# RQLuo/CDLNet-video

Measured on AMD Instinct MI355X. Metric: Mpix/s denoised (fwd+bwd) at K=30,M=64,P=7, higher is better.
Workload: dtype f32 (split-bf16 x3 MFMA, fp32 accumulate, fp32 storage)

## Files before the change

### cdlnet-video_amd/csrc/cdl_fused2d.hip

```cpp
#include <atomic>
#include <cstdlib>
#include <type_traits>
#include <mutex>
#include <utility>
#include <vector>

#include "cdl_common.h"


namespace {

typedef __attribute__((ext_vector_type(8))) __bf16 bf16x8;
typedef __attribute__((ext_vector_type(4))) __bf16 bf16x4;
typedef __attribute__((ext_vector_type(16))) float f32x16;

constexpr int WX = 2;
constexpr int RB = 8;
constexpr int TW = 32 * WX;
constexpr int HALO = 3;
constexpr int RTW = TW + 2 * HALO;
constexpr int RTC = RTW + 2;
constexpr int LDS_W = 32 * 64 * 16;
constexpr int LDS_TAU = 64 * 4;

// ... 115 lines not shown
#endif
#ifndef CDL_FAT_ST_AUX
#define CDL_FAT_ST_AUX 0
#endif
__device__ __forceinline__ __amdgpu_buffer_rsrc_t fat_rsrc(const float *base, size_t img_floats)
{
    return __builtin_amdgcn_make_buffer_rsrc(const_cast<float *>(base), 0, (int)(img_floats * 4), 0x00020000);
}
__device__ __forceinline__ float buf_ld(__amdgpu_buffer_rsrc_t r, int voff, int soff)
{
    return __builtin_bit_cast(float, __builtin_amdgcn_raw_buffer_load_b32(r, voff, soff, CDL_FAT_LD_AUX));
}
__device__ __forceinline__ void buf_st(float v, __amdgpu_buffer_rsrc_t r, int voff, int soff)
{
    __builtin_amdgcn_raw_buffer_store_b32(__builtin_bit_cast(unsigned, v), r, voff, soff, CDL_FAT_ST_AUX);
}
constexpr int OOB = 0x7fff0000;

enum { LAY_NCHW = 0, LAY_BLK = 1, LAY_BLK16 = 2 };
typedef __attribute__((ext_vector_type(4))) unsigned u32x4;
typedef __attribute__((ext_vector_type(2))) unsigned u32x2;

__host__ __device__ inline size_t blk_image_elems(int M, int H, int W) { return (size_t)H * ((W + 31) / 32) * M * 32; }
template <int LAY> __host__ __device__ inline size_t lay_image_bytes(int M, int H, int W)
{
    return LAY == LAY_NCHW ? (size_t)M * H * W * 4 : blk_image_elems(M, H, W) * (LAY == LAY_BLK ? 4 : 2);
}

__device__ __forceinline__ __amdgpu_buffer_rsrc_t uniform_rsrc(const void *base, size_t bytes)
{
    const unsigned long long a = reinterpret_cast<unsigned long long>(base);
    const unsigned lo = __builtin_amdgcn_readfirstlane((unsigned)a);
    const unsigned hi = __builtin_amdgcn_readfirstlane((unsigned)(a >> 32));
    void *b = reinterpret_cast<void *>(((unsigned long long)hi << 32) | lo);
    return __builtin_amdgcn_make_buffer_rsrc(b, 0, __builtin_amdgcn_readfirstlane((int)bytes), 0x00020000);
}

__device__ __forceinline__ float bf16_round(float v) { return (float)(__bf16)v; }

template <int MT>
__device__ __forceinline__ void blk16_load_raw(u32x2 (&z)[MT][4], __amdgpu_buffer_rsrc_t rs, int voff)
{
#pragma unroll
    for (int R = 0; R < MT; ++R)
#pragma unroll
        for (int q = 0; q < 4; ++q)
            z[R][q] = __builtin_bit_cast(u32x2, __builtin_amdgcn_raw_buffer_load_b64(rs, voff, (8 * R + 2 * q) * 32 * 8, CDL_FAT_LD_AUX));
}
__device__ __forceinline__ float blk16_decode(const u32x2 &u, int e)
{
    const unsigned w = (e & 2) ? u.y : u.x;
    return __builtin_bit_cast(float, (e & 1) ? (w & 0xffff0000u) : (w << 16));
}

template <int LAY, int MT>
__device__ __forceinline__ void blk_load(float (&z)[MT][16], __amdgpu_buffer_rsrc_t rs, int voff)
{
    constexpr int EB = LAY == LAY_BLK ? 16 : 8;
#pragma unroll
    for (int R = 0; R < MT; ++R)
#pragma unroll
        for (int q = 0; q < 4; ++q) {
            const int soff = (8 * R + 2 * q) * 32 * EB;
            if constexpr (LAY == LAY_BLK) {
                typedef __attribute__((ext_vector_type(4))) float f32x4;
                const f32x4 f = __builtin_bit_cast(f32x4, __builtin_amdgcn_raw_buffer_load_b128(rs, voff, soff, CDL_FAT_LD_AUX));
                z[R][4 * q + 0] = f.x; z[R][4 * q + 1] = f.y; z[R][4 * q + 2] = f.z; z[R][4 * q + 3] = f.w;
            } else {
                const u32x2 u = __builtin_bit_cast(u32x2, __builtin_amdgcn_raw_buffer_load_b64(rs, voff, soff, CDL_FAT_LD_AUX));
                z[R][4 * q + 0] = __builtin_bit_cast(float, u.x << 16);
                z[R][4 * q + 1] = __builtin_bit_cast(float, u.x & 0xffff0000u);
                z[R][4 * q + 2] = __builtin_bit_cast(float, u.y << 16);
                z[R][4 * q + 3] = __builtin_bit_cast(float, u.y & 0xffff0000u);
            }
        }
}
template <int LAY>
__device__ __forceinline__ void blk_store4(float a0, float a1, float a2, float a3, __amdgpu_buffer_rsrc_t rs, int voff, int quad_pair)
{
    constexpr int EB = LAY == LAY_BLK ? 16 : 8;
    const int soff = quad_pair * 32 * EB;
    if constexpr (LAY == LAY_BLK) {
        typedef __attribute__((ext_vector_type(4))) float f32x4;
        const f32x4 f = {a0, a1, a2, a3};
        __builtin_amdgcn_raw_buffer_store_b128(__builtin_bit_cast(u32x4, f), rs, voff, soff, CDL_FAT_ST_AUX);
    } else {
        u32x2 u;
        u.x = (__builtin_bit_cast(unsigned, a0) >> 16) | (__builtin_bit_cast(unsigned, a1) & 0xffff0000u);
        u.y = (__builtin_bit_cast(unsigned, a2) >> 16) | (__builtin_bit_cast(unsigned, a3) & 0xffff0000u);
        __builtin_amdgcn_raw_buffer_store_b64(u, rs, voff, soff, CDL_FAT_ST_AUX);
    }
}

template <int N>
struct LaneTransposeSum {
    static __device__ __forceinline__ float run(const float (&v)[N], int c)
    {
        constexpr int n = N / 2;
        const bool up = (c & n) != 0;
        float w[n];
#pragma unroll
        for (int k = 0; k < n; ++k) {
            const float keep = up ? v[k + n] : v[k];
            const float send = up ? v[k] : v[k + n];
            w[k] = keep + __shfl_xor(send, n, 64);
        }
        return LaneTransposeSum<n>::run(w, c);
    }
};
template <>
struct LaneTransposeSum<1> {
    static __device__ __forceinline__ float run(const float (&v)[1], int) { return v[0]; }
};
template <int N>
__device__ __forceinline__ float lane_transpose_sum(const float (&v)[N], int c)
{
    float r = LaneTransposeSum<N>::run(v, c);
    if (N == 16) r += __shfl_xor(r, 16, 64);
    return r;
}

__device__ __forceinline__ float wave_shr1(float v)
{
    return __builtin_bit_cast(float, __builtin_amdgcn_update_dpp(0, __builtin_bit_cast(int, v), 0x138, 0xf, 0xf, true));
}
__device__ __forceinline__ float upper_half_to_lower(float v)
{
    float lo = 0.0f;
    asm volatile("s_nop 1\n\tv_permlane32_swap_b32 %0, %1\n\ts_nop 1" : "+v"(v), "+v"(lo));
    return lo;
}
__device__ __forceinline__ float col2im_row(const float (&rv)[4], int h)
{
    const float r4 = upper_half_to_lower(rv[0]);
    const float r5 = upper_half_to_lower(rv[1]);
    const float r6 = upper_half_to_lower(rv[2]);
    const bool lo = h == 0;
    float s = lo ? r6 : 0.0f;
    s = wave_shr1(s) + (lo ? r5 : 0.0f);
    s = wave_shr1(s) + (lo ? r4 : 0.0f);
    s = wave_shr1(s) + (lo ? rv[3] : 0.0f);
    s = wave_shr1(s) + (lo ? rv[2] : 0.0f);
    s = wave_shr1(s) + (lo ? rv[1] : 0.0f);
    s = wave_shr1(s) + (lo ? rv[0] : 0.0f);
    return s;
}

template <int MT, int PREC, int MODE, int LIN, int LOUT, bool DA = false, int WY = 2>
__global__ __launch_bounds__(Shape<WY>::NT) void k_stage(FusedParams p)
{
    using G = Shape<WY>;
    constexpr int NW = G::NW, NT = G::NT, TH = G::TH, RTH = G::RTH, PITCH = G::PITCH, COPY = G::COPY, SLAB = G::SLAB;
    constexpr int LDS_RT = G::LDS_RT, LDS_RSUM = G::LDS_RSUM, LDS_STAGE = G::LDS_STAGE, LDS_DA_THIN = G::LDS_DA_THIN;
    static_assert(!DA || (MODE == MODE_BWD && TH == GW_TH), "dA_k rides in the reverse stage, on k_wgrad2d's 64 x 16 tiles");
    extern __shared__ __attribute__((aligned(16))) unsigned char smem[];
    __bf16 *rt = reinterpret_cast<__bf16 *>(smem);
    float *rsum_all = reinterpret_cast<float *>(smem + LDS_RT);
    const uint4 *wl = reinterpret_cast<const uint4 *>(smem + LDS_RT + LDS_RSUM);
    float *tau_s = reinterpret_cast<float *>(smem + LDS_RT + LDS_RSUM + LDS_W);
    float *tacc_s = tau_s + 64;
    __bf16 *thin2 = reinterpret_cast<__bf16 *>(smem + LDS_STAGE);
    __bf16 *imgs2 = reinterpret_cast<__bf16 *>(smem + LDS_STAGE + LDS_DA_THIN);

    constexpr int M = 32 * MT;
    constexpr int FA = MT * 4, FB = 4 * MT;
    constexpr int NFRAG = (PREC != 1 ? 2 : 1) * (FA + FB);
    constexpr int NSTG = G::NSTG;
    const int tid = threadIdx.x, lane = tid & 63, wid = tid >> 6;
    const int wxi = wid % WX, wyi = wid / WX;
    const int c = lane & 31, h = lane >> 5;
    const size_t HW = (size_t)p.H * p.W;
    const int numTiles = p.N * p.tilesY * p.tilesX;

    {
        uint4 *z4 = reinterpret_cast<uint4 *>(smem);
        for (int i = tid; i < (LDS_RT + LDS_RSUM) / 16; i += NT) z4[i] = make_uint4(0, 0, 0, 0);
        uint4 *wdst = reinterpret_cast<uint4 *>(smem + LDS_RT + LDS_RSUM);
        if (PREC != 1) {
            for (int i = tid; i < NFRAG * 64; i += NT) wdst[i] = p.frags[i];
        } else {
            for (int i = tid; i < FA * 64; i += NT) wdst[i] = p.frags[i];
            for (int i = tid; i < FB * 64; i += NT) wdst[FA * 64 + i] = p.frags[2 * FA * 64 + i];
        }
    }
    float stg[NSTG];
    auto stage_load = [&](int t) {
        int bid = p.rev ? numTiles - 1 - t : t;
        const int txi = bid % p.tilesX; bid /= p.tilesX;
        const int tyi = bid % p.tilesY;
        const int n = bid / p.tilesY;
        const float *rimg = p.r + (size_t)n * HW;
#pragma unroll
        for (int k = 0; k < NSTG; ++k) {
            const int i = tid + k * NT;
            const int yy = i / RTW, xx = i % RTW;
            const int gy = tyi * TH - HALO + yy, gx = txi * TW - HALO + xx;
            float v = 0.0f;
            if (i < RTH * RTW && t < numTiles && !CDL_DBG(p.dbg, 8) && gy >= 0 && gy < p.H && gx >= 0 && gx < p.W)
                v = rimg[(size_t)gy * p.W + gx];
            stg[k] = v;
        }
    };
    auto stage_store = [&]() {
#pragma unroll
        for (int k = 0; k < NSTG; ++k) {
            const int i = tid + k * NT;
            if (i >= RTH * RTW) continue;
            const int yy = i / RTW, xx = i % RTW;
            const __bf16 hh = (__bf16)stg[k];
            const __bf16 ll = (__bf16)(stg[k] - (float)hh);
#pragma unroll
            for (int q = 0; q < 4; ++q)
                if (yy - q >= 0) {
                    rt[(0 * 4 + q) * COPY + xx * PITCH + (yy - q)] = hh;
                    if (PREC != 1) rt[(1 * 4 + q) * COPY + xx * PITCH + (yy - q)] = ll;
                }
        }
    };
    constexpr int NSTG2 = DA ? (GW_RTH * RTW + NT - 1) / NT : 1;
    float stg2[NSTG2];
    auto stage2_load = [&](int t) {
        int bid = p.rev ? numTiles - 1 - t : t;
        const int txi = bid % p.tilesX; bid /= p.tilesX;
        const int tyi = bid % p.tilesY;
        const int n = bid / p.tilesY;
        const float *timg = p.r2 + (t < numTiles ? (size_t)n * HW : 0);
#pragma unroll
        for (int k = 0; k < NSTG2; ++k) {
            const int i = tid + k * NT;
            const int yy = i / RTW, xx = i % RTW;
            const int gy = tyi * TH - HALO + yy, gx = txi * TW - HALO + xx;
            const bool ok = i < GW_RTH * RTW && t < numTiles && gy >= 0 && gy < p.H && gx >= 0 && gx < p.W;
            const float v = timg[ok ? (size_t)gy * p.W + gx : 0];
            stg2[k] = ok ? v : 0.0f;
        }
    };
    auto stage2_store = [&]() {
#pragma unroll
        for (int k = 0; k < NSTG2; ++k) {
            const int i = tid + k * NT;
            if (i >= GW_RTH * RTW) continue;
            const int yy = i / RTW, xx = i % RTW;
            const __bf16 hh = (__bf16)stg2[k];
            const __bf16 ll = (__bf16)(stg2[k] - (float)hh);
#pragma unroll
            for (int sft = 0; sft < 4; ++sft)
                if (xx - sft >= 0) {
                    thin2[(0 * 4 + sft) * TCOPY + yy * TPITCH + xx - sft] = hh;
                    if (PREC != 1) thin2[(1 * 4 + sft) * TCOPY + yy * TPITCH + xx - sft] = ll;
                }
        }
    };
    f32x16 dacc[DA ? MT : 1][2];
    if constexpr (DA) {
#pragma unroll
        for (int R = 0; R < MT; ++R)
#pragma unroll
            for (int tt = 0; tt < 2; ++tt)
#pragma unroll
                for (int v = 0; v < 16; ++v) dacc[R][tt][v] = 0.0f;
        for (int i = tid; i < LDS_DA_THIN / 16; i += NT) reinterpret_cast<uint4 *>(thin2)[i] = make_uint4(0, 0, 0, 0);
        stage2_load(blockIdx.x);
    }
    stage_load(blockIdx.x);
    __syncthreads();
    stage_store();
    if constexpr (DA) stage2_store();

    constexpr int OFF_AH = 0;
    constexpr int OFF_AL = FA;
    constexpr int OFF_BH = (PREC != 1 ? 2 * FA : FA);
    constexpr int OFF_BL = 2 * FA + FB;
    constexpr bool WREG = G::WREG;
    bf16x8 wreg[WREG ? NFRAG : 1];
    if constexpr (WREG) {
#pragma unroll
        for (int f = 0; f < NFRAG; ++f) wreg[f] = __builtin_bit_cast(bf16x8, wl[f * 64 + lane]);
    }
    auto wfrag = [&](int f) __attribute__((always_inline)) {
        if constexpr (WREG) return wreg[f];
        else return __builtin_bit_cast(bf16x8, wl[f * 64 + lane]);
    };

    const int xl = wxi * 32 + c;
    float *rsum = rsum_all + ((wxi & 1) + 2 * (wyi & 1)) * SLAB;
    const bool has_base = (MODE == MODE_FWD) || (MODE == MODE_BWD && p.zin != nullptr);
    const int hw4 = (int)HW * 4;

#pragma unroll 1
    for (int t = blockIdx.x; t < numTiles; t += gridDim.x) {
    const int tile = p.rev ? numTiles - 1 - t : t;
    int bid = tile;
    const int txi = bid % p.tilesX; bid /= p.tilesX;
    const int tyi = bid % p.tilesY;
    const int n = bid / p.tilesY;
    const int tx0 = txi * TW, ty0 = tyi * TH;
    const int x = tx0 + xl;
    if (MODE != MODE_BWD && tid < M) tau_s[tid] = p.tau[(size_t)n * M + tid];
    __syncthreads();
    if (MODE != MODE_BWD) stage_load(t + gridDim.x);

    float ring[7][4];
#pragma unroll
    for (int i = 0; i < 7; ++i)
#pragma unroll
        for (int j = 0; j < 4; ++j) ring[i][j] = 0.0f;
    float tsum[MT * 16];
#pragma unroll
    for (int i = 0; i < MT * 16; ++i) tsum[i] = 0.0f;
    const bool tau_neg = MODE != MODE_BWD && __ballot(lane < M && !(tau_s[lane] >= 0.0f)) != 0ull;
    float taur[MT * 16];
    if (MODE != MODE_BWD) {
#pragma unroll
        for (int R = 0; R < MT; ++R)
#pragma unroll
            for (int qv = 0; qv < 4; ++qv) {
                const float4 t4 = *reinterpret_cast<const float4 *>(&tau_s[32 * R + 8 * qv + 4 * h]);
                taur[16 * R + 4 * qv + 0] = t4.x; taur[16 * R + 4 * qv + 1] = t4.y;
                taur[16 * R + 4 * qv + 2] = t4.z; taur[16 * R + 4 * qv + 3] = t4.w;
            }
    }

    const bool xok = x < p.W;
    const size_t img_in = lay_image_bytes<LIN>(M, p.H, p.W), img_out = lay_image_bytes<LOUT>(M, p.H, p.W);
    const __amdgpu_buffer_rsrc_t rs_in = uniform_rsrc(
        has_base ? (const char *)p.zin + (size_t)n * img_in : (const char *)p.zout, has_base ? img_in : 0);
    unsigned *const map_n = p.map ? p.map + ((size_t)n * 4 + 2 * h) * HW : nullptr;
    const __amdgpu_buffer_rsrc_t rs_out = uniform_rsrc((const char *)p.zout + (size_t)n * img_out, img_out);
    const int lane_off = (int)((4 * h) * HW + x) * 4;
    const int XB = (p.W + 31) / 32, xb = (tx0 >> 5) + wxi;
    constexpr int EB_IN = LIN == LAY_BLK16 ? 8 : 16, EB_OUT = LOUT == LAY_BLK16 ? 8 : 16;
    const int lane_blk_in = (h * 32 + c) * EB_IN, lane_blk_out = (h * 32 + c) * EB_OUT;

#pragma unroll 1
    for (int b = 0; b < RB; ++b) {
        const int yl = wyi * RB + b;
        const int y = ty0 + yl;
        const bool valid = xok && (y < p.H);
        const int voff = valid ? lane_off + y * p.W * 4 : OOB;
        const int blk = (y * XB + xb) * (M / 4) * 32;
        const int voff_in = LIN == LAY_NCHW ? voff : (valid ? blk * EB_IN + lane_blk_in : OOB);
        const int voff_st = CDL_DBG(p.dbg, 1) ? OOB : (LOUT == LAY_NCHW ? voff : (valid ? blk * EB_OUT + lane_blk_out : OOB));

        float zc[MT][16];
        u32x2 zr[MT][4];
        if (MODE != MODE_FIRST && LIN == LAY_BLK16) {
            blk16_load_raw<MT>(zr, rs_in, voff_in);
        } else if (MODE != MODE_FIRST && CDL_DBG(p.dbg, 16)) {
#pragma unroll
            for (int R = 0; R < MT; ++R)
#pragma unroll
                for (int v = 0; v < 16; ++v) zc[R][v] = 0.25f;
        } else if (MODE != MODE_FIRST && LIN != LAY_NCHW) {
            blk_load<LIN, MT>(zc, rs_in, voff_in);
        } else if (MODE != MODE_FIRST) {
#pragma unroll
            for (int R = 0; R < MT; ++R)
#pragma unroll
                for (int v = 0; v < 16; ++v) {
                    const int soff = (32 * R + 8 * (v >> 2) + (v & 3)) * hw4;
                    zc[R][v] = buf_ld(rs_in, voff, soff);
                }
        }
        unsigned sup = 0, sgb = 0;
        if (MODE == MODE_BWD && valid) {
            sup = map_n[(size_t)y * p.W + x];
            sgb = map_n[HW + (size_t)y * p.W + x];
        }

        const int q = b & 3, e = yl - q;
        bf16x8 rh[4], rl[4];
#pragma unroll
        for (int ks = 0; ks < 4; ++ks) {
            const int col = xl + 2 * ks + h;
            const __bf16 *ph = rt + (0 * 4 + q) * COPY + col * PITCH + e;
            const bf16x4 a0 = *reinterpret_cast<const bf16x4 *>(ph);
            const bf16x4 a1 = *reinterpret_cast<const bf16x4 *>(ph + 4);
            rh[ks] = __builtin_shufflevector(a0, a1, 0, 1, 2, 3, 4, 5, 6, 7);
            if (PREC != 1) {
                const __bf16 *pl = rt + (1 * 4 + q) * COPY + col * PITCH + e;
                const bf16x4 b0 = *reinterpret_cast<const bf16x4 *>(pl);
                const bf16x4 b1 = *reinterpret_cast<const bf16x4 *>(pl + 4);
                rl[ks] = __builtin_shufflevector(b0, b1, 0, 1, 2, 3, 4, 5, 6, 7);
            }
        }

        __builtin_amdgcn_sched_barrier(0);
        f32x16 acc[MT];
#pragma unroll
        for (int R = 0; R < MT; ++R)
#pragma unroll
            for (int v = 0; v < 16; ++v) acc[R][v] = 0.0f;
        if CDL_DBG(p.dbg, 4) {
#pragma unroll
            for (int R = 0; R < MT; ++R) acc[R][0] = (float)rh[0][0] + (float)rl[1][1];
        } else {
            bf16x8 wh[2][MT], wlo[2][MT];
#pragma unroll
            for (int R = 0; R < MT; ++R) {
                wh[0][R] = wfrag(OFF_AH + R * 4);
                if (PREC != 1) wlo[0][R] = wfrag(OFF_AL + R * 4);
            }
#pragma unroll
            for (int ks = 0; ks < 4; ++ks) {
                const int cu = ks & 1, nx = cu ^ 1;
                if (ks + 1 < 4) {
#pragma unroll
                    for (int R = 0; R < MT; ++R) {
                        wh[nx][R] = wfrag(OFF_AH + R * 4 + ks + 1);
                        if (PREC != 1) wlo[nx][R] = wfrag(OFF_AL + R * 4 + ks + 1);
                    }
                }
                if (PREC != 1) {
#pragma unroll
                    for (int R = 0; R < MT; ++R) acc[R] = __builtin_amdgcn_mfma_f32_32x32x16_bf16(wlo[cu][R], rh[ks], acc[R], 0, 0, 0);
#pragma unroll
                    for (int R = 0; R < MT; ++R) acc[R] = __builtin_amdgcn_mfma_f32_32x32x16_bf16(wh[cu][R], rl[ks], acc[R], 0, 0, 0);
                    if (PREC == 2) {
#pragma unroll
                        for (int R = 0; R < MT; ++R) acc[R] = __builtin_amdgcn_mfma_f32_32x32x16_bf16(wlo[cu][R], rl[ks], acc[R], 0, 0, 0);
                    }
                }
#pragma unroll
                for (int R = 0; R < MT; ++R) acc[R] = __builtin_amdgcn_mfma_f32_32x32x16_bf16(wh[cu][R], rh[ks], acc[R], 0, 0, 0);
            }
        }

        __builtin_amdgcn_sched_barrier(0);
        auto epilogue = [&](auto general_shrink) {
#pragma unroll
        for (int R = 0; R < MT; ++R)
#pragma unroll
            for (int v = 0; v < 16; ++v) {
                const int chl = 32 * R + 8 * (v >> 2) + (v & 3);
                float zz;
                float zbase = 0.0f;
                if (MODE != MODE_FIRST) zbase = LIN == LAY_BLK16 ? blk16_decode(zr[R][v >> 2], v & 3) : zc[R][v];
                if (MODE == MODE_BWD) {
                    const bool on = (sup >> (16 * R + v)) & 1u;
                    zz = on ? zbase + acc[R][v] : 0.0f;
                    tsum[16 * R + v] += ((sgb >> (16 * R + v)) & 1u) ? zz : -zz;
                } else {
                    const float base = (MODE == MODE_FWD) ? zbase : 0.0f;
                    const float u = fmaf(p.sgn, acc[R][v], base);
                    const float tt = taur[16 * R + v];
                    const float st = decltype(general_shrink)::value ? cdl_shrink(u, tt)
                                                                     : u - __builtin_amdgcn_fmed3f(u, -tt, tt);
                    zz = CDL_DBG(p.dbg, 64) ? u : (valid ? st : 0.0f);
                }
                if (LOUT == LAY_BLK16) zz = bf16_round(zz);
                if (LOUT == LAY_NCHW) buf_st(zz, rs_out, voff_st, chl * hw4);
                acc[R][v] = zz;
            }
        };
        if (tau_neg) epilogue(std::true_type{});
        else epilogue(std::false_type{});
        if (LOUT != LAY_NCHW) {
#pragma unroll
            for (int R = 0; R < MT; ++R)
#pragma unroll
                for (int q = 0; q < 4; ++q)
                    blk_store4<LOUT>(acc[R][4 * q], acc[R][4 * q + 1], acc[R][4 * q + 2], acc[R][4 * q + 3], rs_out,
                                     voff_st, 8 * R + 2 * q);
        }
        if (MODE != MODE_BWD && map_n) {
            unsigned ws = 0, wg = 0;
#pragma unroll
            for (int R = 0; R < MT; ++R)
#pragma unroll
                for (int v = 0; v < 16; ++v) {
                    const float zz = acc[R][v];
                    ws |= (zz != 0.0f ? 1u : 0u) << (16 * R + v);
                    wg |= (__builtin_bit_cast(unsigned, zz) >> 31) << (16 * R + v);
                }
            if (valid && !CDL_DBG(p.dbg, 1)) {
                map_n[(size_t)y * p.W + x] = ws;
                map_n[HW + (size_t)y * p.W + x] = wg;
            }
        }
        if constexpr (DA) {
            __bf16 *wimg = imgs2 + (size_t)wid * (MT * 2) * IMG_ELEMS;
#pragma unroll
            for (int R = 0; R < MT; ++R)
#pragma unroll
                for (int qv = 0; qv < 4; ++qv) {
                    bf16x4 hi4, lo4;
#pragma unroll
                    for (int e = 0; e < 4; ++e) {
                        const float val = acc[R][4 * qv + e];
                        const __bf16 hh = (__bf16)val;
                        hi4[e] = hh;
                        lo4[e] = (__bf16)(val - (float)hh);
                    }
                    const int slot = (2 * qv + h) ^ ((c >> 1) & 7);
                    __bf16 *dst = wimg + (size_t)(R * 2) * IMG_ELEMS + c * 32 + slot * 4;
                    *reinterpret_cast<bf16x4 *>(dst) = hi4;
                    if (PREC != 1 && LOUT != LAY_BLK16) *reinterpret_cast<bf16x4 *>(dst + IMG_ELEMS) = lo4;
                }
            __builtin_amdgcn_fence(__ATOMIC_RELEASE, "wavefront");
            __builtin_amdgcn_wave_barrier();
#pragma unroll
            for (int kk = 0; kk < 2; ++kk) {
                bf16x8 Bh[2], Bl[2];
#pragma unroll
                for (int tt = 0; tt < 2; ++tt) {
                    const int tap = 32 * tt + c, ti = tap >> 3, tj = tap & 7;
                    const int e0 = wxi * 32 + 16 * kk + 8 * h + (tj & 4);
                    const __bf16 *ph = thin2 + (0 * 4 + (tj & 3)) * TCOPY + (yl + ti) * TPITCH + e0;
                    const bf16x4 a0 = *reinterpret_cast<const bf16x4 *>(ph);
                    const bf16x4 a1 = *reinterpret_cast<const bf16x4 *>(ph + 4);
                    Bh[tt] = __builtin_shufflevector(a0, a1, 0, 1, 2, 3, 4, 5, 6, 7);
                    if (PREC != 1) {
                        const __bf16 *pl = ph + 4 * TCOPY;
                        const bf16x4 b0 = *reinterpret_cast<const bf16x4 *>(pl);
                        const bf16x4 b1 = *reinterpret_cast<const bf16x4 *>(pl + 4);
                        Bl[tt] = __builtin_shufflevector(b0, b1, 0, 1, 2, 3, 4, 5, 6, 7);
                    }
                }
#pragma unroll
                for (int R = 0; R < MT; ++R) {
                    const int gg = (lane >> 4) & 1, qq = (lane >> 2) & 3, pp = lane & 3;
                    bf16x4 part[2][2];
#pragma unroll
                    for (int half = 0; half < 2; ++half) {
                        const int row = 16 * kk + 8 * h + 4 * half + qq;
                        const int slot = (4 * gg + pp) ^ ((row >> 1) & 7);
                        const __bf16 *src = wimg + (size_t)(R * 2) * IMG_ELEMS + row * 32 + slot * 4;
                        part[0][half] = __builtin_amdgcn_ds_read_tr16_b64_v4bf16(
                            (__attribute__((address_space(3))) bf16x4 *)(src));
                        if (PREC != 1 && LOUT != LAY_BLK16)
                            part[1][half] = __builtin_amdgcn_ds_read_tr16_b64_v4bf16(
                                (__attribute__((address_space(3))) bf16x4 *)(src + IMG_ELEMS));
                    }
                    const bf16x8 Ah = __builtin_shufflevector(part[0][0], part[0][1], 0, 1, 2, 3, 4, 5, 6, 7);
                    bf16x8 Al;
                    if (PREC != 1 && LOUT != LAY_BLK16) Al = __builtin_shufflevector(part[1][0], part[1][1], 0, 1, 2, 3, 4, 5, 6, 7);
#pragma unroll
                    for (int tt = 0; tt < 2; ++tt) {
                        if (PREC != 1) {
                            if (LOUT != LAY_BLK16) dacc[R][tt] = __builtin_amdgcn_mfma_f32_32x32x16_bf16(Al, Bh[tt], dacc[R][tt], 0, 0, 0);
                            dacc[R][tt] = __builtin_amdgcn_mfma_f32_32x32x16_bf16(Ah, Bl[tt], dacc[R][tt], 0, 0, 0);
                            if (PREC == 2 && LOUT != LAY_BLK16) dacc[R][tt] = __builtin_amdgcn_mfma_f32_32x32x16_bf16(Al, Bl[tt], dacc[R][tt], 0, 0, 0);
                        }
                        dacc[R][tt] = __builtin_amdgcn_mfma_f32_32x32x16_bf16(Ah, Bh[tt], dacc[R][tt], 0, 0, 0);
                    }
                }
            }
            __builtin_amdgcn_fence(__ATOMIC_RELEASE, "wavefront");
            __builtin_amdgcn_wave_barrier();
        }
        if (MODE == MODE_BWD && !p.do_synth) continue;
        if CDL_DBG(p.dbg, 2) { ring[0][0] += acc[0][0] + acc[MT - 1][15]; continue; }

        __builtin_amdgcn_sched_barrier(0);
        f32x16 D[2];
#pragma unroll
        for (int Rp = 0; Rp < 2; ++Rp)
#pragma unroll
            for (int v = 0; v < 16; ++v) D[Rp][v] = 0.0f;
        {
            bf16x8 bwh[2][2], bwl[2][2];
#pragma unroll
            for (int Rp = 0; Rp < 2; ++Rp) {
                bwh[0][Rp] = wfrag(OFF_BH + Rp * 2 * MT);
                if (PREC != 1) bwl[0][Rp] = wfrag(OFF_BL + Rp * 2 * MT);
            }
#pragma unroll
            for (int q = 0; q < 2 * MT; ++q) {
                const int R = q >> 1, s = q & 1, cu = q & 1, nx = cu ^ 1;
                if (q + 1 < 2 * MT) {
#pragma unroll
                    for (int Rp = 0; Rp < 2; ++Rp) {
                        bwh[nx][Rp] = wfrag(OFF_BH + Rp * 2 * MT + q + 1);
                        if (PREC != 1) bwl[nx][Rp] = wfrag(OFF_BL + Rp * 2 * MT + q + 1);
                    }
                }
                bf16x8 zh, zl;
#pragma unroll
                for (int jj = 0; jj < 8; ++jj) {
                    const float val = acc[R][8 * s + jj];
                    const __bf16 hh = (__bf16)val;
                    zh[jj] = hh;
                    if (PREC != 1 && LOUT != LAY_BLK16) zl[jj] = (__bf16)(val - (float)hh);
                }
                if (PREC != 1) {
#pragma unroll
                    for (int Rp = 0; Rp < 2; ++Rp) D[Rp] = __builtin_amdgcn_mfma_f32_32x32x16_bf16(bwl[cu][Rp], zh, D[Rp], 0, 0, 0);
                    if (LOUT != LAY_BLK16) {
#pragma unroll
                        for (int Rp = 0; Rp < 2; ++Rp) D[Rp] = __builtin_amdgcn_mfma_f32_32x32x16_bf16(bwh[cu][Rp], zl, D[Rp], 0, 0, 0);
                        if (PREC == 2) {
#pragma unroll
                            for (int Rp = 0; Rp < 2; ++Rp) D[Rp] = __builtin_amdgcn_mfma_f32_32x32x16_bf16(bwl[cu][Rp], zl, D[Rp], 0, 0, 0);
                        }
                    }
                }
#pragma unroll
                for (int Rp = 0; Rp < 2; ++Rp) D[Rp] = __builtin_amdgcn_mfma_f32_32x32x16_bf16(bwh[cu][Rp], zh, D[Rp], 0, 0, 0);
            }
        }

        __builtin_amdgcn_sched_barrier(0);
#pragma unroll
        for (int Rp = 0; Rp < 2; ++Rp)
#pragma unroll
            for (int v = 0; v < 16; ++v) {
                const int i = 4 * Rp + (v >> 2);
                if (i <= 6) ring[i][v & 3] += D[Rp][v];
            }
        {
            const float cs = col2im_row(ring[0], h);
            if (lane < 38 && !CDL_DBG(p.dbg, 32)) rsum[yl * RTW + 32 * wxi + lane] = cs;
        }
#pragma unroll
        for (int i = 0; i < 6; ++i)
#pragma unroll
            for (int jl = 0; jl < 4; ++jl) ring[i][jl] = ring[i + 1][jl];
#pragma unroll
        for (int jl = 0; jl < 4; ++jl) ring[6][jl] = 0.0f;
    }

    if (MODE != MODE_BWD || p.do_synth) {
#pragma unroll
        for (int i = 0; i < 6; ++i) {
            const float cs = col2im_row(ring[i], h);
            if (lane < 38 && !CDL_DBG(p.dbg, 32)) rsum[(wyi * RB + RB + i) * RTW + 32 * wxi + lane] = cs;
        }
    }
    if (MODE == MODE_BWD) {
        const float tacc = lane_transpose_sum(tsum, c);
        if (c < MT * 16) {
            const int R = c >> 4, v = c & 15;
            tacc_s[wid * 64 + 32 * R + 8 * (v >> 2) + 4 * h + (v & 3)] = tacc;
        }
    }
    __syncthreads();
    if (MODE == MODE_BWD) stage_load(t + gridDim.x);
    if constexpr (DA) stage2_load(t + gridDim.x);
    if (MODE == MODE_BWD && tid < M) {
        float sacc = 0.0f;
#pragma unroll
        for (int w = 0; w < NW; ++w) sacc += tacc_s[w * 64 + tid];
        p.dtau[(size_t)tile * M + tid] = sacc;
    }
    if (MODE != MODE_BWD || p.do_synth) {
        float *patch = p.patches + (size_t)tile * SLAB;
        for (int i = tid; i < SLAB; i += NT) {
            patch[i] = (rsum_all[i] + rsum_all[SLAB + i]) + (rsum_all[2 * SLAB + i] + rsum_all[3 * SLAB + i]);
            rsum_all[i] = 0.0f; rsum_all[SLAB + i] = 0.0f; rsum_all[2 * SLAB + i] = 0.0f; rsum_all[3 * SLAB + i] = 0.0f;
        }
    }
    stage_store();
    if constexpr (DA) stage2_store();
    }
    if constexpr (DA) {
        float *red = reinterpret_cast<float *>(smem);
        for (int w = 0; w < NW; ++w) {
            __syncthreads();
            if (wid == w) {
#pragma unroll
                for (int R = 0; R < MT; ++R)
#pragma unroll
                    for (int tt = 0; tt < 2; ++tt)
#pragma unroll
                        for (int v = 0; v < 16; ++v) {
                            const int ch = 32 * R + (v & 3) + 8 * (v >> 2) + 4 * h;
                            float *dstw = &red[ch * 64 + 32 * tt + c];
                            *dstw = (w == 0 ? 0.0f : *dstw) + dacc[R][tt][v];
                        }
            }
        }
        __syncthreads();
        float *dst = p.da_partial + (size_t)blockIdx.x * 2 * M * 64;
        for (int i = tid; i < M * 64; i += NT) dst[i] = red[i];
    }
}

template <int WY>
__device__ __forceinline__ float patch_sum(const float *__restrict__ patches, int n, int Y, int X,
                                           int tilesX, int tilesY)
{
    constexpr int TH = Shape<WY>::TH, SLAB = Shape<WY>::SLAB;
    const int tyc = Y / TH, txc = X / TW;
    const int ly = Y - tyc * TH, lx = X - txc * TW;
    const int hx = (lx < HALO && txc > 0) ? -1 : ((lx >= TW - HALO && txc + 1 < tilesX) ? 1 : 0);
    const int vy = (ly < HALO && tyc > 0) ? -1 : ((ly >= TH - HALO && tyc + 1 < tilesY) ? 1 : 0);
    const float *own = patches + (((size_t)n * tilesY + tyc) * tilesX + txc) * SLAB + (ly + HALO) * RTW + lx + HALO;
    const ptrdiff_t dx = (ptrdiff_t)hx * (SLAB - TW), dy = (ptrdiff_t)vy * ((ptrdiff_t)tilesX * SLAB - TH * RTW);
    float sum = 0.0f;
    if (vy < 0) {
        if (hx < 0) sum += own[dy + dx];
        sum += own[dy];
        if (hx > 0) sum += own[dy + dx];
    }
    if (hx < 0) sum += own[dx];
    sum += own[0];
    if (hx > 0) sum += own[dx];
    if (vy > 0) {
        if (hx < 0) sum += own[dy + dx];
        sum += own[dy];
        if (hx > 0) sum += own[dy + dx];
    }
    return sum;
}

template <int ASM_ROWS, int WY>
__global__ __launch_bounds__(256) void k_assemble(const float *__restrict__ patches,
                                                  const float *__restrict__ mask,
                                                  const float *__restrict__ sub, float alpha,
                                                  float *__restrict__ out, int N, int H, int W,
                                                  int tilesX, int tilesY, float *__restrict__ acc, int acc_add)
{
    const int X = blockIdx.x * 256 + threadIdx.x, n = blockIdx.z;
    if (X >= W) return;
#pragma unroll
    for (int j = 0; j < ASM_ROWS; ++j) {
        const int Y = blockIdx.y * ASM_ROWS + j;
        if (Y >= H) break;
        const size_t i = ((size_t)n * H + Y) * W + X;
        const float raw = patch_sum<WY>(patches, n, Y, X, tilesX, tilesY);
        if (acc) acc[i] = acc_add ? acc[i] + raw : raw;
        if (!out) continue;
        float sum = alpha * raw;
        if (mask) sum *= mask[i];
        if (sub) sum -= sub[i];
        out[i] = sum;
    }
}

template <int WY>
__global__ __launch_bounds__(256) void k_assemble_v4(const float *__restrict__ patches,
                                                     const float *__restrict__ mask, const float *__restrict__ sub,
                                                     float alpha, float *__restrict__ out, int N, int H, int W,
                                                     int tilesX, int tilesY, float *__restrict__ accum, int acc_add)
{
    constexpr int TH = Shape<WY>::TH, SLAB = Shape<WY>::SLAB;
    const int X = (blockIdx.x * 64 + (threadIdx.x & 63)) * 4, n = blockIdx.z;
    if (X >= W) return;
    const int txc = X / TW, lx = X - txc * TW;
// ... 1019 lines not shown
```

### cdlnet-video_amd/ops.py

```python
import ctypes
from dataclasses import dataclass
from typing import Optional, Tuple

import torch

from . import _lib


def _stream():
    return ctypes.c_void_p(torch.cuda.current_stream().cuda_stream)


def _first_cuda_tensor(args, kwargs=None):
    for a in list(args) + (list(kwargs.values()) if kwargs else []):
        if torch.is_tensor(a):
            if a.is_cuda:
                return a
        elif isinstance(a, (list, tuple)):
            t = _first_cuda_tensor(a)
            if t is not None:
                return t
    return None


# ... 621 lines not shown
    if layout == "nchw":
        return z
    H, W = g.dims[1], g.dims[2]
    XB = (W + 31) // 32
    zp = torch.nn.functional.pad(z, (0, XB * 32 - W))
    v = zp.reshape(g.N, g.M // 4, 4, H, XB, 32).permute(0, 3, 4, 1, 5, 2).contiguous().reshape(1, -1)
    return v[0].to(torch.bfloat16 if layout == "blocked_bf16" else torch.float32)


def fused_supported(g: Geometry) -> bool:
    gs = g.c_struct()
    return bool(_lib.lib().cdl_fused2d_supported(ctypes.byref(gs)))


def fused_prep(wA, wB):
    wA, wB = _dev(wA, "wA"), _dev(wB, "wB")
    M, P = wA.shape[0], wA.shape[-1]
    nbytes = _lib.lib().cdl_fused2d_frag_bytes(M)
    frags = torch.empty(nbytes, device=wA.device, dtype=torch.uint8)
    rc = _lib.lib().cdl_fused2d_prep(_ptr(wA), _ptr(wB), _ptr(frags), M, P, _stream())
    _lib.check(rc, "cdl_fused2d_prep")
    return frags


def fused_patches(g: Geometry, device):
    gs = g.c_struct()
    n = _lib.lib().cdl_fused2d_patch_floats(ctypes.byref(gs))
    return torch.empty(n, device=device, dtype=torch.float32)


def fused_map(g: Geometry, device):
    gs = g.c_struct()
    n = int(_lib.lib().cdl_fused2d_map_words(ctypes.byref(gs)))
    assert n == g.N * 4 * g.dims[1] * g.dims[2]
    return torch.empty((g.N, 4, g.dims[1], g.dims[2]), device=device, dtype=torch.int32)


def fused_support_map(g: Geometry, z, out=None):
    z = _dev(z, "z")
    assert tuple(z.shape) == g.code_shape()
    if out is None:
        out = fused_map(g, z.device)
    gs = g.c_struct()
    rc = _lib.lib().cdl_fused2d_support_map(ctypes.byref(gs), _ptr(z), _ptr(out), _stream())
    _lib.check(rc, "cdl_fused2d_support_map")
    return out


def fused_iter(g: Geometry, r, zin, tau, frags, sgn, patches, precision="split3", out=None, map_out=None,
               lay_in="nchw", lay_out="nchw"):
    r, tau = _dev(r, "r"), _dev(tau, "tau")
    if zin is not None and lay_in == "nchw":
        zin = _dev(zin, "zin")
    assert tuple(r.shape) == g.image_shape()
    if out is None:
        out = fused_code_buffer(g, lay_out, r.device)[0]
    gs = g.c_struct()
    rc = _lib.lib().cdl_fused2d_iter_fwd(ctypes.byref(gs), _ptr(r), _ptr(zin), _ptr(tau), _ptr(frags),
                                         float(sgn), _ptr(out), _ptr(patches), _ptr(map_out),
                                         PRECISION[precision] | _lay_in(lay_in) | _lay_out(lay_out), _stream())
    _lib.check(rc, "cdl_fused2d_iter_fwd")
    return out


def fused_assemble(g: Geometry, patches, mask=None, sub=None, alpha=1.0, out=None, acc=None, acc_add=False,
                   write_out=True):
    mask, sub = _opt(mask, "mask"), _opt(sub, "sub")
    assert acc is None or (acc.is_contiguous() and tuple(acc.shape) == g.image_shape())
    if write_out and out is None:
        out = torch.empty(g.image_shape(), device=patches.device, dtype=torch.float32)
    rc = _lib.lib().cdl_fused2d_assemble(ctypes.byref(g.c_struct()), _ptr(patches), _ptr(mask), _ptr(sub),
                                         float(alpha), _ptr(out if write_out else None), _ptr(acc),
                                         int(bool(acc_add)), _stream())
    _lib.check(rc, "cdl_fused2d_assemble")
    return out if write_out else None


def fused_tiles(g: Geometry) -> int:
    gs = g.c_struct()
    return int(_lib.lib().cdl_fused2d_tiles(ctypes.byref(gs)))


def fused_stage_bwd(g: Geometry, thin, base, gate, frags, patches, dtau_partial, do_synth,
                    precision="split3", out=None, lay_in="nchw", lay_out="nchw", r2=None, alpha=1.0, workspace=None):
    thin = _dev(thin, "thin")
    if base is not None and lay_in == "nchw":
        base = _dev(base, "base")
    if gate.dtype != torch.int32:
        gate = fused_support_map(g, gate)
    assert gate.is_cuda and gate.is_contiguous() and gate.numel() == g.N * 4 * g.dims[1] * g.dims[2]
    if out is None:
        out = fused_code_buffer(g, lay_out, thin.device)[0]
    gs = g.c_struct()
    flags = PRECISION[precision] | _lay_in(lay_in) | _lay_out(lay_out)
    r2 = _opt(r2, "r2")
    dA = None if r2 is None else torch.empty(g.filter_shape(), device=thin.device, dtype=torch.float32)
    rc = _lib.lib().cdl_fused2d_stage_bwd(ctypes.byref(gs), _ptr(thin), _ptr(base), _ptr(gate), _ptr(frags), _ptr(out),
                                          _ptr(patches), _ptr(dtau_partial), int(bool(do_synth)), _ptr(r2),
                                          float(alpha), _ptr(dA), _ptr(workspace), flags, _stream())
    _lib.check(rc, "cdl_fused2d_stage_bwd")
    return out if dA is None else (out, dA)


def fused_dtau_reduce(g: Geometry, dtau_partial, c, dt_k, dtau_n=None):
    assert dt_k.is_contiguous() and dt_k.numel() == 2 * g.M
    assert dtau_n is None or (dtau_n.is_contiguous() and dtau_n.numel() == g.N * g.M)
    gs = g.c_struct()
    base = dt_k.data_ptr()
    rc = _lib.lib().cdl_fused2d_dtau_reduce(ctypes.byref(gs), _ptr(dtau_partial), _ptr(_opt(c, "c")),
                                            ctypes.c_void_p(base), ctypes.c_void_p(base + 4 * g.M), _ptr(dtau_n),
                                            _stream())
    _lib.check(rc, "cdl_fused2d_dtau_reduce")


def fused_wgrad_workspace(g: Geometry, device):
    gs = g.c_struct()
    n = _lib.lib().cdl_fused2d_wgrad_workspace_floats(ctypes.byref(gs))
    return torch.empty(n, device=device, dtype=torch.float32)


def fused_wgrad(g: Geometry, workspace, X0=None, T0=None, alpha0=1.0, X1=None, T1=None, alpha1=1.0,
                precision="split3", layout="nchw", tiles_reversed=False):
    outs = []
    args = []
    for X, T, al in ((X0, T0, alpha0), (X1, T1, alpha1)):
        if X is None:
            outs.append(None)
            args += [None, None, 0.0, None]
        else:
            X, T = (_dev(X, "X") if layout == "nchw" else X), _dev(T, "T")
            dw = torch.empty(g.filter_shape(), device=X.device, dtype=torch.float32)
            outs.append(dw)
            args += [_ptr(X), _ptr(T), float(al), _ptr(dw)]
    gs = g.c_struct()
    rc = _lib.lib().cdl_fused2d_wgrad(ctypes.byref(gs), *args, _ptr(workspace),
                                      PRECISION[precision] | _lay_in(layout) | (TILES_REVERSED if tiles_reversed else 0),
                                      _stream())
    _lib.check(rc, "cdl_fused2d_wgrad")
    return outs


def _check_data_grads(g: Geometry, K, dyp, dtau):
    for t, shape in ((dyp, g.image_shape()), (dtau, (K, g.N, g.M))):
        if t is not None:
            assert t.is_cuda and t.dtype == torch.float32 and t.is_contiguous() and tuple(t.shape) == tuple(shape), \
                (tuple(t.shape), shape)


def _ptr_table(tensors):
    return (ctypes.c_void_p * len(tensors))(*[t.data_ptr() for t in tensors])


def fused_forward(g: Geometry, yp, mask_p, tau, A, B, keep, precision="split3", layout="blocked", keep_maps=False):
    K = len(A)
    yp, tau = _dev(yp, "yp"), _dev(tau, "tau")
    mask_p = _opt(mask_p, "mask")
    A = [_dev(w, "A") for w in A]
    B = [_dev(w, "B") for w in B]
    dev = yp.device
    nz = (K - 1) if keep else min(K - 1, 2)
    nr = (K - 1) if keep else min(K - 1, 2)
    zK = torch.empty(g.code_shape(), device=dev, dtype=torch.float32)
    zbuf = fused_code_buffer(g, layout, dev, max(nz, 1))
    rbuf = torch.empty((max(nr, 1),) + g.image_shape(), device=dev, dtype=torch.float32)
    z = [zbuf[k % nz] for k in range(K - 1)] + [zK]
    r = [rbuf[k % nr] for k in range(K - 1)] if K > 1 else []
    maps = list(torch.empty((K, g.N, 4, g.dims[1], g.dims[2]), device=dev, dtype=torch.int32).unbind(0)) \
        if (keep or keep_maps) else []
    xp = torch.empty(g.image_shape(), device=dev, dtype=torch.float32)
    frags = torch.empty(K * _lib.lib().cdl_fused2d_frag_bytes(g.M), device=dev, dtype=torch.uint8)
    patches = fused_patches(g, dev)
    gs = g.c_struct()
    rc = _lib.lib().cdl_fused2d_forward(ctypes.byref(gs), K, _ptr(yp), _ptr(mask_p), _ptr(tau), _ptr_table(A),
                                        _ptr_table(B), _ptr_table(z), _ptr_table(r) if r else None,
                                        _ptr_table(maps) if maps else None, _ptr(xp), _ptr(frags), _ptr(patches),
                                        PRECISION[precision] | _lay_in(layout), _stream())
    _lib.check(rc, "cdl_fused2d_forward")
# ... 437 lines not shown
```

Baseline: 119.9.

## Hand-schedule DA backward stage by interleaving MFMA chains with epilogue and LDS reads

In the dA-fused reverse stage, the analysis MFMAs, the epilogue, the transposed LDS reads, the dA_k MFMAs, the tau-gradient sums and the synthesis MFMAs are woven together. This uses compile-time static_for, inline-asm pinned MFMAs and sched_barriers so VALU/LDS work sits in the shadow of MFMA chains. The goal is to hide the serial gaps between accumulation, epilogue and the dA/synthesis matmuls. In exchange, the inline asm with hand-placed s_nops bypasses the compiler's hazard handling, which raises correctness and register-pressure risk. The ops.py side also gains a tiles_reversed flag, though the TILES_REVERSED constant is not visibly defined.

```diff
diff --git a/cdlnet-video_amd/csrc/cdl_fused2d.hip b/cdlnet-video_amd/csrc/cdl_fused2d.hip
--- a/cdlnet-video_amd/csrc/cdl_fused2d.hip
+++ b/cdlnet-video_amd/csrc/cdl_fused2d.hip
@@ -221,8 +221,9 @@
     const int soff = quad_pair * 32 * EB;
     if constexpr (LAY == LAY_BLK) {
         typedef __attribute__((ext_vector_type(4))) float f32x4;
-        const f32x4 f = {a0, a1, a2, a3};
-        __builtin_amdgcn_raw_buffer_store_b128(__builtin_bit_cast(u32x4, f), rs, voff, soff, CDL_FAT_ST_AUX);
+        const u32x4 d = __builtin_bit_cast(u32x4, (f32x4){a0, a1, a2, a3});
+        __builtin_amdgcn_raw_buffer_store_b128(d, rs, voff, soff, CDL_FAT_ST_AUX);
+        asm volatile("s_nop 1" : : "v"(d));
     } else {
         u32x2 u;
         u.x = (__builtin_bit_cast(unsigned, a0) >> 16) | (__builtin_bit_cast(unsigned, a1) & 0xffff0000u);
@@ -285,6 +286,26 @@
     return s;
 }
 
+template <int... I, class F>
+__device__ __forceinline__ void static_for_seq(std::integer_sequence<int, I...>, F &&f)
+{
+    (f(std::integral_constant<int, I>{}), ...);
+}
+template <int N, class F>
+__device__ __forceinline__ void static_for(F &&f) { static_for_seq(std::make_integer_sequence<int, N>{}, f); }
+
+__device__ __forceinline__ void mfma_pinned(f32x16 &C, const bf16x8 &A, const bf16x8 &B)
+{
+    asm volatile("s_nop 1\n\tv_mfma_f32_32x32x16_bf16 %0, %1, %2, %0" : "+a"(C) : "v"(A), "v"(B) : "memory");
+}
+__device__ __forceinline__ void mfma_pinned_first(f32x16 &C, const bf16x8 &A, const bf16x8 &B)
+{
+    asm volatile("s_nop 1\n\tv_mfma_f32_32x32x16_bf16 %0, %1, %2, 0" : "=&a"(C) : "v"(A), "v"(B) : "memory");
+}
+__device__ __forceinline__ void mfma_chain_end(f32x16 &C) { asm volatile("s_nop 15" : "+a"(C)); }
+template <class T> __device__ __forceinline__ void pin_value(T &x) { asm volatile("" : "+v"(x)); }
+template <class T> __device__ __forceinline__ void pin_values(T &x, T &y) { asm volatile("" : "+v"(x), "+v"(y)); }
+
 template <int MT, int PREC, int MODE, int LIN, int LOUT, bool DA = false, int WY = 2>
 __global__ __launch_bounds__(Shape<WY>::NT) void k_stage(FusedParams p)
 {
@@ -341,9 +362,11 @@
         }
     };
     auto stage_store = [&]() {
+        int tid_t = tid;
+        if constexpr (DA) pin_value(tid_t);
 #pragma unroll
         for (int k = 0; k < NSTG; ++k) {
-            const int i = tid + k * NT;
+            const int i = tid_t + k * NT;
             if (i >= RTH * RTW) continue;
             const int yy = i / RTW, xx = i % RTW;
             const __bf16 hh = (__bf16)stg[k];
@@ -375,9 +398,11 @@
         }
     };
     auto stage2_store = [&]() {
+        int tid_t = tid;
+        pin_value(tid_t);
 #pragma unroll
         for (int k = 0; k < NSTG2; ++k) {
-            const int i = tid + k * NT;
+            const int i = tid_t + k * NT;
             if (i >= GW_RTH * RTW) continue;
             const int yy = i / RTW, xx = i % RTW;
             const __bf16 hh = (__bf16)stg2[k];
@@ -526,6 +551,7 @@
 
         __builtin_amdgcn_sched_barrier(0);
         f32x16 acc[MT];
+        if constexpr (!DA) {
 #pragma unroll
         for (int R = 0; R < MT; ++R)
 #pragma unroll
@@ -563,6 +589,7 @@
 #pragma unroll
                 for (int R = 0; R < MT; ++R) acc[R] = __builtin_amdgcn_mfma_f32_32x32x16_bf16(wh[cu][R], rh[ks], acc[R], 0, 0, 0);
             }
+        }
         }
 
         __builtin_amdgcn_sched_barrier(0);
@@ -592,9 +619,11 @@
                 acc[R][v] = zz;
             }
         };
+        if constexpr (!DA) {
         if (tau_neg) epilogue(std::true_type{});
         else epilogue(std::false_type{});
-        if (LOUT != LAY_NCHW) {
+        }
+        if (!DA && LOUT != LAY_NCHW) {
 #pragma unroll
             for (int R = 0; R < MT; ++R)
 #pragma unroll
@@ -617,48 +646,84 @@
                 map_n[HW + (size_t)y * p.W + x] = wg;
             }
         }
+        f32x16 D[2];
         if constexpr (DA) {
+            constexpr int NP = PREC == 1 ? 1 : (PREC == 2 ? 4 : 3);
+            constexpr bool ZLO = PREC != 1 && LOUT != LAY_BLK16;
+            constexpr int NPZ = ZLO ? NP : (PREC != 1 ? 2 : 1);
+            constexpr int NA = 4 * NP, NZ = 4 * NPZ;
+            constexpr bool TS_LATE = LOUT != LAY_BLK16;
             __bf16 *wimg = imgs2 + (size_t)wid * (MT * 2) * IMG_ELEMS;
-#pragma unroll
-            for (int R = 0; R < MT; ++R)
-#pragma unroll
-                for (int qv = 0; qv < 4; ++qv) {
-                    bf16x4 hi4, lo4;
-#pragma unroll
-                    for (int e = 0; e < 4; ++e) {
-                        const float val = acc[R][4 * qv + e];
-                        const __bf16 hh = (__bf16)val;
-                        hi4[e] = hh;
-                        lo4[e] = (__bf16)(val - (float)hh);
-                    }
+            float zz[MT][16];
+            bf16x4 zh4[MT][4], zl4[MT][4];
+            bf16x8 Bh[2][2], Bl[2][2];
+            bf16x8 Ah[2], Al[2];
+
+            auto ana = [&](auto Rc, auto mc) __attribute__((always_inline)) {
+                constexpr int R = decltype(Rc)::value, m = decltype(mc)::value, ks = m / NP, j = m % NP;
+                constexpr bool whi = j == NP - 1 || j == 1, rhi = j == NP - 1 || j == 0;
+                const bf16x8 w = wfrag((whi ? OFF_AH : OFF_AL) + R * 4 + ks);
+                if constexpr (m == 0) mfma_pinned_first(acc[R], w, rhi ? rh[ks] : rl[ks]);
+                else mfma_pinned(acc[R], w, rhi ? rh[ks] : rl[ks]);
+            };
+            auto epi = [&](auto Rc, auto vc) __attribute__((always_inline)) {
+                constexpr int R = decltype(Rc)::value, v = decltype(vc)::value, qv = v >> 2;
+                if constexpr (v == 0) mfma_chain_end(acc[R]);
+                const float zbase = LIN == LAY_BLK16 ? blk16_decode(zr[R][qv], v & 3) : zc[R][v];
+                const bool on = (sup >> (16 * R + v)) & 1u;
+                float z = on ? zbase + acc[R][v] : 0.0f;
+                if constexpr (!TS_LATE) {
+                    tsum[16 * R + v] += ((sgb >> (16 * R + v)) & 1u) ? z : -z;
+                    z = bf16_round(z);
+                }
+                if (LOUT == LAY_NCHW) buf_st(z, rs_out, voff_st, (32 * R + 8 * qv + (v & 3)) * hw4);
+                const __bf16 hh = (__bf16)z;
+                zh4[R][qv][v & 3] = hh;
+                if constexpr (ZLO) zl4[R][qv][v & 3] = (__bf16)(z - (float)hh);
+                zz[R][v] = z;
+                if constexpr ((v & 3) == 3) {
+                    if (LOUT != LAY_NCHW)
+                        blk_store4<LOUT>(zz[R][v - 3], zz[R][v - 2], zz[R][v - 1], zz[R][v], rs_out, voff_st, 8 * R + 2 * qv);
                     const int slot = (2 * qv + h) ^ ((c >> 1) & 7);
                     __bf16 *dst = wimg + (size_t)(R * 2) * IMG_ELEMS + c * 32 + slot * 4;
-                    *reinterpret_cast<bf16x4 *>(dst) = hi4;
-                    if (PREC != 1 && LOUT != LAY_BLK16) *reinterpret_cast<bf16x4 *>(dst + IMG_ELEMS) = lo4;
+                    *reinterpret_cast<bf16x4 *>(dst) = zh4[R][qv];
+                    if constexpr (ZLO) *reinterpret_cast<bf16x4 *>(dst + IMG_ELEMS) = zl4[R][qv];
+                } else if constexpr ((v & 3) == 1) {
+                    pin_values(zz[R][v - 1], zz[R][v]);
                 }
-            __builtin_amdgcn_fence(__ATOMIC_RELEASE, "wavefront");
-            __builtin_amdgcn_wave_barrier();
-#pragma unroll
-            for (int kk = 0; kk < 2; ++kk) {
-                bf16x8 Bh[2], Bl[2];
-#pragma unroll
-                for (int tt = 0; tt < 2; ++tt) {
-                    const int tap = 32 * tt + c, ti = tap >> 3, tj = tap & 7;
-                    const int e0 = wxi * 32 + 16 * kk + 8 * h + (tj & 4);
-                    const __bf16 *ph = thin2 + (0 * 4 + (tj & 3)) * TCOPY + (yl + ti) * TPITCH + e0;
-                    const bf16x4 a0 = *reinterpret_cast<const bf16x4 *>(ph);
-                    const bf16x4 a1 = *reinterpret_cast<const bf16x4 *>(ph + 4);
-                    Bh[tt] = __builtin_shufflevector(a0, a1, 0, 1, 2, 3, 4, 5, 6, 7);
-                    if (PREC != 1) {
-                        const __bf16 *pl = ph + 4 * TCOPY;
-                        const bf16x4 b0 = *reinterpret_cast<const bf16x4 *>(pl);
-                        const bf16x4 b1 = *reinterpret_cast<const bf16x4 *>(pl + 4);
-                        Bl[tt] = __builtin_shufflevector(b0, b1, 0, 1, 2, 3, 4, 5, 6, 7);
+            };
+            auto tgrad = [&](auto uc) __attribute__((always_inline)) {
+                constexpr int u = 2 * decltype(uc)::value;
+                tsum[u] += ((sgb >> u) & 1u) ? zz[u >> 4][u & 15] : -zz[u >> 4][u & 15];
+                tsum[u + 1] += ((sgb >> (u + 1)) & 1u) ? zz[u >> 4][(u & 15) + 1] : -zz[u >> 4][(u & 15) + 1];
+                pin_values(tsum[u], tsum[u + 1]);
+            };
+            auto thin_reads = [&]() __attribute__((always_inline)) {
+#pragma unroll
+                for (int kk = 0; kk < 2; ++kk)
+#pragma unroll
+                    for (int tt = 0; tt < 2; ++tt) {
+                        const int tap = 32 * tt + c, ti = tap >> 3, tj = tap & 7;
+                        const int e0 = wxi * 32 + 16 * kk + 8 * h + (tj & 4);
+                        const __bf16 *ph = thin2 + (0 * 4 + (tj & 3)) * TCOPY + (yl + ti) * TPITCH + e0;
+                        const bf16x4 a0 = *reinterpret_cast<const bf16x4 *>(ph);
+                        const bf16x4 a1 = *reinterpret_cast<const bf16x4 *>(ph + 4);
+                        Bh[kk][tt] = __builtin_shufflevector(a0, a1, 0, 1, 2, 3, 4, 5, 6, 7);
+                        if (PREC != 1) {
+                            const __bf16 *pl = ph + 4 * TCOPY;
+                            const bf16x4 b0 = *reinterpret_cast<const bf16x4 *>(pl);
+                            const bf16x4 b1 = *reinterpret_cast<const bf16x4 *>(pl + 4);
+                            Bl[kk][tt] = __builtin_shufflevector(b0, b1, 0, 1, 2, 3, 4, 5, 6, 7);
+                        }
                     }
-                }
-#pragma unroll
-                for (int R = 0; R < MT; ++R) {
-                    const int gg = (lane >> 4) & 1, qq = (lane >> 2) & 3, pp = lane & 3;
+            };
+            auto tr_reads = [&](auto Rc) __attribute__((always_inline)) {
+                constexpr int R = decltype(Rc)::value;
+                __builtin_amdgcn_fence(__ATOMIC_RELEASE, "wavefront");
+                __builtin_amdgcn_wave_barrier();
+                const int gg = (lane >> 4) & 1, qq = (lane >> 2) & 3, pp = lane & 3;
+#pragma unroll
+                for (int kk = 0; kk < 2; ++kk) {
                     bf16x4 part[2][2];
 #pragma unroll
                     for (int half = 0; half < 2; ++half) {
@@ -667,32 +732,82 @@
                         const __bf16 *src = wimg + (size_t)(R * 2) * IMG_ELEMS + row * 32 + slot * 4;
                         part[0][half] = __builtin_amdgcn_ds_read_tr16_b64_v4bf16(
                             (__attribute__((address_space(3))) bf16x4 *)(src));
-                        if (PREC != 1 && LOUT != LAY_BLK16)
+                        if constexpr (ZLO)
                             part[1][half] = __builtin_amdgcn_ds_read_tr16_b64_v4bf16(
                                 (__attribute__((address_space(3))) bf16x4 *)(src + IMG_ELEMS));
                     }
-                    const bf16x8 Ah = __builtin_shufflevector(part[0][0], part[0][1], 0, 1, 2, 3, 4, 5, 6, 7);
-                    bf16x8 Al;
-                    if (PREC != 1 && LOUT != LAY_BLK16) Al = __builtin_shufflevector(part[1][0], part[1][1], 0, 1, 2, 3, 4, 5, 6, 7);
-#pragma unroll
-                    for (int tt = 0; tt < 2; ++tt) {
-                        if (PREC != 1) {
-                            if (LOUT != LAY_BLK16) dacc[R][tt] = __builtin_amdgcn_mfma_f32_32x32x16_bf16(Al, Bh[tt], dacc[R][tt], 0, 0, 0);
-                            dacc[R][tt] = __builtin_amdgcn_mfma_f32_32x32x16_bf16(Ah, Bl[tt], dacc[R][tt], 0, 0, 0);
-                            if (PREC == 2 && LOUT != LAY_BLK16) dacc[R][tt] = __builtin_amdgcn_mfma_f32_32x32x16_bf16(Al, Bl[tt], dacc[R][tt], 0, 0, 0);
-                        }
-                        dacc[R][tt] = __builtin_amdgcn_mfma_f32_32x32x16_bf16(Ah, Bh[tt], dacc[R][tt], 0, 0, 0);
-                    }
+                    Ah[kk] = __builtin_shufflevector(part[0][0], part[0][1], 0, 1, 2, 3, 4, 5, 6, 7);
+                    if constexpr (ZLO) Al[kk] = __builtin_shufflevector(part[1][0], part[1][1], 0, 1, 2, 3, 4, 5, 6, 7);
                 }
+            };
+            auto dak = [&](auto Rc, auto mc) __attribute__((always_inline)) {
+                constexpr int R = decltype(Rc)::value, m = decltype(mc)::value;
+                constexpr int kk = m / (2 * NPZ), j = (m / 2) % NPZ, tt = m % 2;
+                constexpr bool duhi = !ZLO || j == NPZ - 1 || j == 1, thi = j == NPZ - 1 || (ZLO && j == 0);
+                mfma_pinned(dacc[R][tt], duhi ? Ah[kk] : Al[kk], thi ? Bh[kk][tt] : Bl[kk][tt]);
+            };
+            auto syn = [&](auto Rc, auto mc) __attribute__((always_inline)) {
+                constexpr int R = decltype(Rc)::value, m = decltype(mc)::value;
+                constexpr int s = m / (2 * NPZ), j = (m / 2) % NPZ, Rp = m % 2, q = 2 * R + s;
+                constexpr bool whi = j == NPZ - 1 || (ZLO && j == 1), zhi = !ZLO || j == NPZ - 1 || j == 0;
+                const bf16x8 w = wfrag((whi ? OFF_BH : OFF_BL) + Rp * 2 * MT + q);
+                const bf16x8 zq = zhi ? __builtin_shufflevector(zh4[R][2 * s], zh4[R][2 * s + 1], 0, 1, 2, 3, 4, 5, 6, 7)
+                                      : __builtin_shufflevector(zl4[R][2 * s], zl4[R][2 * s + 1], 0, 1, 2, 3, 4, 5, 6, 7);
+                if constexpr (R == 0 && m < 2) mfma_pinned_first(D[Rp], w, zq);
+                else mfma_pinned(D[Rp], w, zq);
+            };
+            auto beside = [&](auto NMc, auto NMUc, auto NUc, auto &&mf, auto &&unit) __attribute__((always_inline)) {
+                constexpr int NM = decltype(NMc)::value, NMU = decltype(NMUc)::value, NU = decltype(NUc)::value;
+                static_for<NM>([&](auto mc) __attribute__((always_inline)) {
+                    constexpr int m = decltype(mc)::value;
+                    mf(mc);
+                    constexpr int lo = m < NMU ? NU * m / NMU : NU, hi = m + 1 < NMU ? NU * (m + 1) / NMU : NU;
+                    static_for<hi - lo>([&](auto dc) __attribute__((always_inline)) {
+                        unit(std::integral_constant<int, lo + decltype(dc)::value>{});
+                    });
+                    __builtin_amdgcn_sched_barrier(0);
+                });
+            };
+            using std::integral_constant;
+            constexpr integral_constant<int, 0> T0{};
+            constexpr integral_constant<int, MT - 1> T1{};
+            auto nothing = [&](auto) __attribute__((always_inline)) {};
+
+            __builtin_amdgcn_sched_barrier(0);
+            beside(integral_constant<int, NA>{}, T0, T0, [&](auto mc) __attribute__((always_inline)) { ana(T0, mc); }, nothing);
+            if constexpr (MT == 2) {
+                beside(integral_constant<int, NA>{}, integral_constant<int, NA * 3 / 4>{}, integral_constant<int, 17>{},
+                       [&](auto mc) __attribute__((always_inline)) { ana(T1, mc); },
+                       [&](auto uc) __attribute__((always_inline)) {
+                           if constexpr (decltype(uc)::value < 16) epi(T0, uc);
+                           else { tr_reads(T0); thin_reads(); }
+                       });
+                beside(integral_constant<int, NZ>{}, integral_constant<int, NZ>{}, integral_constant<int, 16>{},
+                       [&](auto mc) __attribute__((always_inline)) { dak(T0, mc); },
+                       [&](auto uc) __attribute__((always_inline)) { epi(T1, uc); });
+                tr_reads(T1);
+                if (p.do_synth)
+                    beside(integral_constant<int, NZ>{}, T0, T0, [&](auto mc) __attribute__((always_inline)) { syn(T0, mc); }, nothing);
+            } else {
+                static_for<16>([&](auto vc) __attribute__((always_inline)) { epi(T0, vc); });
+                tr_reads(T0);
+                thin_reads();
+                __builtin_amdgcn_sched_barrier(0);
             }
+            beside(integral_constant<int, NZ>{}, integral_constant<int, NZ>{}, integral_constant<int, TS_LATE ? 8 * MT : 0>{},
+                   [&](auto mc) __attribute__((always_inline)) { dak(T1, mc); }, tgrad);
             __builtin_amdgcn_fence(__ATOMIC_RELEASE, "wavefront");
             __builtin_amdgcn_wave_barrier();
+            if (!p.do_synth) continue;
+            beside(integral_constant<int, NZ>{}, T0, T0, [&](auto mc) __attribute__((always_inline)) { syn(T1, mc); }, nothing);
+            mfma_chain_end(D[0]);
+            mfma_chain_end(D[1]);
         }
         if (MODE == MODE_BWD && !p.do_synth) continue;
         if CDL_DBG(p.dbg, 2) { ring[0][0] += acc[0][0] + acc[MT - 1][15]; continue; }
 
         __builtin_amdgcn_sched_barrier(0);
-        f32x16 D[2];
+        if constexpr (!DA) {
 #pragma unroll
         for (int Rp = 0; Rp < 2; ++Rp)
 #pragma unroll
@@ -738,6 +853,7 @@
                 for (int Rp = 0; Rp < 2; ++Rp) D[Rp] = __builtin_amdgcn_mfma_f32_32x32x16_bf16(bwh[cu][Rp], zh, D[Rp], 0, 0, 0);
             }
         }
+        }
 
         __builtin_amdgcn_sched_barrier(0);
 #pragma unroll
@@ -794,6 +910,8 @@
     }
     if constexpr (DA) {
         float *red = reinterpret_cast<float *>(smem);
+#pragma unroll
+        for (int R = 0; R < MT; ++R) { mfma_chain_end(dacc[R][0]); mfma_chain_end(dacc[R][1]); }
         for (int w = 0; w < NW; ++w) {
             __syncthreads();
             if (wid == w) {
diff --git a/cdlnet-video_amd/ops.py b/cdlnet-video_amd/ops.py
--- a/cdlnet-video_amd/ops.py
+++ b/cdlnet-video_amd/ops.py
@@ -727,7 +727,8 @@
 
 
 def fused_stage_bwd(g: Geometry, thin, base, gate, frags, patches, dtau_partial, do_synth,
-                    precision="split3", out=None, lay_in="nchw", lay_out="nchw", r2=None, alpha=1.0, workspace=None):
+                    precision="split3", out=None, lay_in="nchw", lay_out="nchw", r2=None, alpha=1.0, workspace=None,
+                    tiles_reversed=False):
     thin = _dev(thin, "thin")
     if base is not None and lay_in == "nchw":
         base = _dev(base, "base")
@@ -737,7 +738,7 @@
     if out is None:
         out = fused_code_buffer(g, lay_out, thin.device)[0]
     gs = g.c_struct()
-    flags = PRECISION[precision] | _lay_in(lay_in) | _lay_out(lay_out)
+    flags = PRECISION[precision] | _lay_in(lay_in) | _lay_out(lay_out) | (TILES_REVERSED if tiles_reversed else 0)
     r2 = _opt(r2, "r2")
     dA = None if r2 is None else torch.empty(g.filter_shape(), device=thin.device, dtype=torch.float32)
     rc = _lib.lib().cdl_fused2d_stage_bwd(ctypes.byref(gs), _ptr(thin), _ptr(base), _ptr(gate), _ptr(frags), _ptr(out),
```

New measurement: 115.9. -3.4%, worse.
